# kazuotani14/iLQR

Measured on AMD Instinct MI355X. Metric: iLQR iterations/sec (batch x T timesteps/sec), acrobot T=500 batch=4096, higher is better.
Workload: dtype f64; 1 GPU; acrobot n=4 m=1 T=499 (500 knots), box-QP limits active, FD derivatives + backward/box-QP + 11-alpha search + accept, fixed work; batch_per_gpu=4096, global_batch=4096, T=499, parallelism=batch shards x1, one all_gather of costs

## Files before the change

ilqr_amd/csrc/backward_hex.hpp:

```cpp
#pragma once
#include "solve_tile.hpp"

namespace ilqr {

#ifndef ILQR_COMMIT_ROLLED
#define ILQR_COMMIT_ROLLED 1
#endif

constexpr int HT = 4;
#ifndef ILQR_HEX_SLOT_PAD
#define ILQR_HEX_SLOT_PAD 8
#endif
#ifndef ILQR_HEX_PAIR_PERM
#define ILQR_HEX_PAIR_PERM 1
#endif
#ifndef ILQR_HEX_CAND_T
#define ILQR_HEX_CAND_T 1
#endif
constexpr bool kHexCandT = ILQR_HEX_CAND_T != 0;

template <int NX, int NU, class real, int SLOTS_, bool COMPACT_ = false>
struct HexRing {
  static constexpr bool COMPACT = COMPACT_;
  static constexpr int US = Rec<NX, NU>::SIZE;
  static constexpr int PAIRS = COMPACT ? CompactRec<NX, NU>::PAIRS : (Rec<NX, NU>::SIZE + NU + 1) / 2;
  static constexpr int ROW = 2 * HT;
  static constexpr int PAD = ROW - 2 * TW;
  static constexpr int ELEMS = PAIRS * ROW + ILQR_HEX_SLOT_PAD;
  static constexpr int Z = PAIRS * ROW;
  static_assert(!COMPACT || ILQR_HEX_SLOT_PAD >= ROW, "the compact slot keeps Z in its pad row");
  static_assert(!COMPACT || (NX == 4 && NU == 1), "compact slots: nx = 4, nu = 1");
  static constexpr int SLOTS = SLOTS_;
  static constexpr bool PERM = (ILQR_HEX_PAIR_PERM != 0) && NX == 4 && NU == 1;
  static constexpr int pos(int pair) { return PERM && (!COMPACT || pair < 8) ? hex_pair_pos(pair) : pair; }
};

constexpr int kHexKnotsPerRound = 64 / HT;
constexpr int kHexFullSlots = 24;
template <int NX, int NU, class real, bool COMPACT>
struct HexRingSize {
  using Full = HexRing<NX, NU, real, kHexFullSlots, false>;
  static constexpr int TERM = COMPACT ? ((NX + NX * NX) / 2) * Full::ROW : 0;
  static constexpr int SLOTS = COMPACT ? (kHexFullSlots * Full::ELEMS - TERM) / HexRing<NX, NU, real, 1, COMPACT>::ELEMS : kHexFullSlots;
  static constexpr int LEAD = SLOTS - kHexKnotsPerRound - 1;
  static_assert(SLOTS > LEAD + kHexKnotsPerRound - 1 && LEAD >= 1, "a round must not reach a slot the chain has not left");
  static_assert(SLOTS * HexRing<NX, NU, real, 1, COMPACT>::ELEMS + TERM <= kHexFullSlots * Full::ELEMS, "the pair's records fit the bytes of 24 full slots");
};

template <class real, int N>
struct HexTerm {
  alignas(16) real term[N];
};
template <class real>
struct HexTerm<real, 0> {
  static constexpr real* term = nullptr;
};

template <class real, int NX, int NU, bool COMPACT = false>
struct HexPair : HexTerm<real, HexRingSize<NX, NU, real, COMPACT>::TERM> {
  using Size = HexRingSize<NX, NU, real, COMPACT>;
  using RS = HexRing<NX, NU, real, Size::SLOTS, COMPACT>;
  static constexpr int LEAD = Size::LEAD;
  alignas(16) real ring[RS::SLOTS * RS::ELEMS];
  int rounds_done;
  int consumer_at;
  int passes_started;
  unsigned long long pass_lanes;
};

template <class P>
struct HexGate {
  static constexpr bool kRing = true;
  P& sh;
  const int T, nrounds, N;
  int pass = -1, have = 0;
  int g_next = 0, slot_next = 0, slot_cur = 0;
  __device__ __forceinline__ HexGate(P& s, int T_) : sh(s), T(T_), nrounds((T_ + 1 + kHexKnotsPerRound - 1) / kHexKnotsPerRound), N(nrounds * kHexKnotsPerRound) {}
  __device__ __forceinline__ void begin_pass() {
    pass++;
    have = pass * N;
    g_next = pass * N;
    slot_next = g_next % P::RS::SLOTS;
    __hip_atomic_store(&sh.pass_lanes, __ballot(1), __ATOMIC_RELAXED, __HIP_MEMORY_SCOPE_WORKGROUP);
    __hip_atomic_store(&sh.passes_started, pass + 1, __ATOMIC_RELEASE, __HIP_MEMORY_SCOPE_WORKGROUP);
  }
  __device__ __forceinline__ int slot(int) const { return slot_cur; }
  __device__ __forceinline__ void wait(int) {
    const int G = g_next++;
    slot_cur = slot_next;
    slot_next = (slot_next + 1 == P::RS::SLOTS) ? 0 : slot_next + 1;
    __hip_atomic_store(&sh.consumer_at, G, __ATOMIC_RELAXED, __HIP_MEMORY_SCOPE_WORKGROUP);
    if (G < have) return;
    const int round = pass * nrounds + (G - pass * N) / kHexKnotsPerRound;
    while (__hip_atomic_load(&sh.rounds_done, __ATOMIC_ACQUIRE, __HIP_MEMORY_SCOPE_WORKGROUP) <= round) __builtin_amdgcn_s_sleep(1);
    have = pass * N + ((G - pass * N) / kHexKnotsPerRound + 1) * kHexKnotsPerRound;
  }
  __device__ __forceinline__ void finish() {
    __hip_atomic_store(&sh.consumer_at, 0x3fffffff, __ATOMIC_RELAXED, __HIP_MEMORY_SCOPE_WORKGROUP);
    __hip_atomic_store(&sh.passes_started, -1, __ATOMIC_RELEASE, __HIP_MEMORY_SCOPE_WORKGROUP);
  }
};

__device__ __forceinline__ int hex_first(unsigned long long bal, int t4) {
  return __builtin_ctzll(((bal >> t4) & 0x000F000F000F000Full) | 0x8000000000000000ull);
}
__device__ __forceinline__ void qp1_search_hex(QP1StateT<double>& q, int j, int t4, double step_j0, const double* __restrict__ lds_steps) {
  const double t_x1 = clamp_of(q.x + step_j0 * q.search, q.lo, q.hi);
  const double t_v1 = qp1_value(q, t_x1);
  const bool t_pass = !qp1_armijo_fails(q, t_v1, step_j0);
  const int pp = hex_first(__ballot(t_pass), t4);
  const bool success = pp < 52;
  const int jw = success ? (((pp >> 4) << 2) | (pp & 3)) : 0;
#ifdef ILQR_EXP_NO_STEP_LDS
  q.step = jw == 0 ? 1.0 : 0.6;
#else
  q.step = lds_steps[jw];
#endif
  q.x1 = clamp_of(q.x + q.step * q.search, q.lo, q.hi);
  q.v1 = qp1_value(q, q.x1);
  bool more = p_and(!success, !q.early);
  if (__builtin_expect(__ballot(more) == 0ull, 1)) return;
  {
    const bool stuck = p_and(j >= 1, t_x1 == q.x);
    const int qs = hex_first(__ballot(p_and(stuck, more)), t4);
    if (p_and(more, qs < 52)) {
      q.ls_failed = true;
      more = false;
    }
    if (__ballot(more) == 0ull) return;
  }
  for (int base = 16;; base += 16) {
    const int kn = base + j;
    const double my_step = lds_steps[kn < 104 ? kn : 103];
    const double my_x1 = qp1_trial(q, my_step);
    const double my_v1 = qp1_value(q, my_x1);
    const bool pass = !qp1_armijo_fails(q, my_v1, my_step);
    const bool stuck = p_or(my_step < kMinStep, my_x1 == q.x);
    const int qp = hex_first(__ballot(p_and(pass, more)), t4), qs = hex_first(__ballot(p_and(stuck, more)), t4);
    if (more) {
      if (qp < qs) {
        q.step = lds_steps[base + (((qp >> 4) << 2) | (qp & 3))];
        q.x1 = qp1_trial(q, q.step);
        q.v1 = qp1_value(q, q.x1);
        more = false;
      } else if (qs < 52) {
        q.ls_failed = true;
        more = false;
      }
    }
    if (__ballot(more) == 0ull) return;
  }
}

template <class RS>
__device__ __forceinline__ int hex_pos_rt(int pair) { return RS::pos(pair); }

template <class real>
struct HexStep {
  typedef real pair_t __attribute__((ext_vector_type(2)));
  real F, cxx_rc, cxx_cr, fu_r, cx_r, cxu_r, cxu_c;
  pair_t tail, uw;
};

template <class M, class Gate, class RS>
__device__ __forceinline__ void backward_hex(const BatchViewT<typename M::real>& v, const M& model, const SolverParams& sp, int mode, int tile, int sub,
                                             int lane, const double* __restrict__ lds_steps, Gate& gate, const typename M::real* __restrict__ ring,
                                             const typename M::real* __restrict__ term ) {
  using real = typename M::real;
  using creal = double;
  static_assert(M::NX == 4 && M::NU == 1, "hex chain: nx = 4, nu = 1");
  using R = Rec<4, 1>;
  typedef real real2_t __attribute__((ext_vector_type(2)));
  const int r_ = lane >> 4, t_ = (lane >> 2) & 3, c_ = lane & 3, j16 = 4 * r_ + c_;
  const int t4 = 4 * t_;
  const int l = sub * HT + t_;
  const int b = tile * TW + l;
  if (b >= v.B) return;
  if (mode == 1 && v.status[b] != 0) return;
  const int T = v.T;
  double lambda = v.lambda[b], dlambda = v.dlambda[b];
  const real* __restrict__ ust = v.us + tidx(tile, 0, 0, l, T, 1);
  real* __restrict__ kt = v.kff + tidx(tile, 0, 0, l, T, 1);
  real* __restrict__ Kt = v.Kfb + tidx(tile, 0, 0, l, T, 4);
  typedef const __attribute__((address_space(3))) real lds_cd;
  typedef const __attribute__((address_space(3))) real2_t lds_cd2;
  const creal step_j0 = lds_steps[j16];
  auto mm = [](creal a, creal bb) __attribute__((always_inline)) { return __builtin_amdgcn_mfma_f64_4x4x4f64(a, bb, 0.0, 0, 0, 0); };

  auto load = [&](int t, HexStep<real>& d) __attribute__((always_inline)) {
    gate.wait(t);
    lds_cd* r = (lds_cd*)(ring + gate.slot(t) * RS::ELEMS + t_ * 2);
    auto pair = [&](int e) { return *(lds_cd2*)(r + RS::pos(e >> 1) * RS::ROW); };
    auto one = [&](int e) { return r[hex_pos_rt<RS>(e >> 1) * RS::ROW + (e & 1)]; };
    if constexpr (RS::COMPACT) {
      using C = CompactRec<4, 1>;
      d.F = one(C::FX + r_ + 4 * c_);
      d.fu_r = one(C::FU + r_);
      d.cxx_rc = d.cxx_cr = d.cx_r = d.cxu_r = d.cxu_c = r[RS::Z];
      d.tail = pair(C::CU);
      d.uw = pair(C::US);
      return;
    }
    d.F = one(R::FX + r_ + 4 * c_);
    d.cxx_rc = one(R::CXX + r_ + 4 * c_);
    d.cxx_cr = one(R::CXX + c_ + 4 * r_);
    d.fu_r = one(R::FU + r_);
    d.cx_r = one(R::CX + r_);
    d.cxu_r = one(R::CXU + r_);
    d.cxu_c = one(R::CXU + c_);
    d.tail = pair(R::CU);
    d.uw = pair(RS::US);
  };

  int diverge = 0;
  bool done = false;
  double dV0 = 0, dV1 = 0, gacc = 0;
  auto one_pass = [&]() __attribute__((always_inline)) {
    gate.begin_pass();
    creal V, RVx, kprev;
    const creal lam_r = (creal)lambda;
    {
      gate.wait(T);
      if constexpr (RS::COMPACT) {
        using C = CompactRec<4, 1>;
        lds_cd* r = (lds_cd*)(term + t_ * 2);
        RVx = (creal)r[((C::TERM_CX + r_) >> 1) * RS::ROW + ((C::TERM_CX + r_) & 1)];
        V = (creal)r[((C::TERM_CXX + r_ + 4 * c_) >> 1) * RS::ROW + ((C::TERM_CXX + r_ + 4 * c_) & 1)];
      } else {
      lds_cd* r = (lds_cd*)(ring + gate.slot(T) * RS::ELEMS + t_ * 2);
      RVx = (creal)r[hex_pos_rt<RS>((R::CX + r_) >> 1) * RS::ROW + ((R::CX + r_) & 1)];
      V = (creal)r[hex_pos_rt<RS>((R::CXX + r_ + 4 * c_) >> 1) * RS::ROW + ((R::CXX + r_ + 4 * c_) & 1)];
      }
    }
    kprev = (creal)kt[(unsigned)((T - 1) * TW)];
    __builtin_amdgcn_s_waitcnt(0x0F70);
    dV0 = dV1 = 0;
    diverge = 0;
    gacc = 0;
    real* __restrict__ Kt_i = Kt + (unsigned)(((T - 1) * 4 + c_) * TW);
    real* __restrict__ kt_i = kt + (unsigned)((T - 1) * TW);

    auto step = [&](int i, const HexStep<real>& raw, HexStep<real>& nxt) -> bool {
      const creal F = (creal)raw.F, Rfu = (creal)raw.fu_r;
      const creal cu = (creal)raw.tail.x, cuu = (creal)raw.tail.y, us = (creal)raw.uw.x, usw = (creal)raw.uw.y;
      const creal W = mm(V, F);
      const creal wv = mm(V, Rfu);
      const creal aQu = mm(Rfu, RVx);
      const creal aQx = mm(F, RVx);
      const creal Tm = mm(F, W);
      const creal Tt = mm(W, F);
      const creal aQuu = mm(Rfu, wv);
      const creal aQux_c = mm(Rfu, W);
      const creal aQux_r = mm(W, Rfu);
      const creal Qxx_rc = (creal)raw.cxx_rc + Tm, Qxx_cr = (creal)raw.cxx_cr + Tt;
      const creal Qx_r = (creal)raw.cx_r + aQx;
      const creal Qu = cu + aQu;
      const creal Qux_c = (creal)raw.cxu_c + aQux_c, Qux_r = (creal)raw.cxu_r + aQux_r;
      const creal Quu = cuu + aQuu, QuuF = (cuu + lam_r) + aQuu;
      const creal lo = (creal)model.u_min[0] - us, hi = (creal)model.u_max[0] - us;
      __builtin_amdgcn_sched_barrier(0);
      if (i >= 1) load(i - 1, nxt);
      __builtin_amdgcn_sched_barrier(0);
      creal x;
      int free0;
      creal minv;
      QP1StateT<creal> q1;
      qp1_begin<false>(QuuF, Qu, kprev, lo, hi, q1, false);
      qp1_search_hex(q1, j16, t4, step_j0, lds_steps);
      bool goes_on;
      bool ok = qp1_finish_ok(q1, x, free0, minv, goes_on);
      if (goes_on)
        ok = qp1_continue(
                 q1, [&](QP1StateT<creal>& qs) __attribute__((always_inline)) { qp1_search_hex(qs, j16, t4, step_j0, lds_steps); }, x, free0) >= 1;
      if (!ok) diverge = i;
      const creal k_scale = free0 ? -minv : creal(0);
      const creal K_r = k_scale * Qux_r, K_c = k_scale * Qux_c;
      creal d0 = 0, d1 = 0;
      {
        d0 += x * Qu;
        creal rq = 0;
        rq += (creal(0.5) * x) * Quu;
        d1 += rq * x;
      }
      creal T1_r, T1_c;
      {
        creal acc = 0;
        acc += K_r * Quu;
        T1_r = acc;
      }
      {
        creal acc = 0;
        acc += K_c * Quu;
        T1_c = acc;
      }
      creal Vxn_r, Vn_rc, Vn_cr;
      {
        creal t1 = 0, t2 = 0, t3 = 0;
        t1 += T1_r * x;
        t2 += K_r * Qu;
        t3 += Qux_r * x;
        Vxn_r = ((Qx_r + t1) + t2) + t3;
      }
      {
        creal u1 = 0, u2 = 0, u3 = 0;
        u1 += T1_r * K_c;
        u2 += K_r * Qux_c;
        u3 += Qux_r * K_c;
        Vn_rc = ((Qxx_rc + u1) + u2) + u3;
      }
      {
        creal u1 = 0, u2 = 0, u3 = 0;
        u1 += T1_c * K_r;
        u2 += K_c * Qux_r;
        u3 += Qux_c * K_r;
        Vn_cr = ((Qxx_cr + u1) + u2) + u3;
      }
      V = creal(0.5) * (Vn_rc + Vn_cr);
      RVx = Vxn_r;
      if (ok) {
        dV0 += (double)d0;
        dV1 += (double)d1;
        gacc += (double)(abs_of(x) * usw);
        kprev = (creal)(real)x;
        Kt_i[0] = (real)K_c;
        kt_i[0] = (real)x;
      }
      Kt_i -= 4 * TW;
      kt_i -= TW;
      return ok;
    };

    HexStep<real> A, Bd;
    int i = T - 1;
    load(i, A);
    while (true) {
      if (!step(i, A, Bd)) break;
      if (--i < 0) break;
      if (!step(i, Bd, A)) break;
      if (--i < 0) break;
    }
  };

  while (true) {
    one_pass();
    if (mode == 0) {
      done = (diverge == 0);
      break;
    }
    if (diverge != 0) {
      dlambda = raised_dlambda(dlambda, sp);
      lambda = raised_lambda(lambda, dlambda, sp);
      if (lambda > sp.lambda_max) break;
      continue;
    }
    done = true;
    break;
  }

  double acc = gacc;
  if (!done) {
    __builtin_amdgcn_fence(__ATOMIC_RELEASE, "workgroup");
    __builtin_amdgcn_s_waitcnt(0);
    acc = 0;
    for (int t0 = 0; t0 < T; t0 += 8) {
      real kv[8], uv[8];
#pragma unroll
      for (int jj = 0; jj < 8; jj++) {
        const int t = (t0 + jj < T) ? t0 + jj : T - 1;
        kv[jj] = kt[(size_t)t * TW];
        uv[jj] = ust[(size_t)t * TW];
      }
#pragma unroll
      for (int jj = 0; jj < 8; jj++) {
        const real mx = abs_of(kv[jj]) / (abs_of(uv[jj]) + 1);
        if (t0 + jj < T) acc += (double)mx;
      }
    }
  }
  const double gnorm = acc / T;
  if (j16 == 0) {
    v.dV[b] = dV0;
    v.dV[v.Bp + b] = dV1;
    v.diverge[b] = diverge;
    v.backpass_done[b] = done ? 1 : 0;
    v.gnorm[b] = gnorm;
    if (mode == 1) {
      v.lambda[b] = lambda;
      v.dlambda[b] = dlambda;
      if (!sp.fixed_work && gnorm < sp.tol_grad && lambda < kLambdaConverged) {
        v.status[b] = 1;
        v.iters[b] += 1;
      }
    }
  }
}

template <class M, class MFD, class P>
__device__ __forceinline__ void sweep_backward_hex(const BatchViewT<typename M::real>& v, const M& model, const MFD& fdm, const SolverParams& sp, int mode,
                                                   int force, int tile, P* pairs, const double* __restrict__ lds_steps, int role) {
  using RS = typename P::RS;
  const int lane = threadIdx.x & 63;
  if (threadIdx.x < 4) {
    pairs[threadIdx.x].rounds_done = 0;
    pairs[threadIdx.x].consumer_at = 0;
    pairs[threadIdx.x].passes_started = 0;
  }
  __syncthreads();
  const int T = v.T;
  P& sh = pairs[role & 3];
  if (role < 4) {
    __builtin_amdgcn_s_setprio(3);
    HexGate<P> gate(sh, T);
    backward_hex<M, decltype(gate), RS>(v, model, sp, mode, tile, role, lane, lds_steps, gate, sh.ring, sh.term);
    gate.finish();
    __builtin_amdgcn_s_setprio(0);
  } else {
    const int sub = role - 4;
    const int lp = lane & (HT - 1), ks = lane >> 2;
    const int l = sub * HT + lp;
    const int nrounds = (T + 1 + kHexKnotsPerRound - 1) / kHexKnotsPerRound, N = nrounds * kHexKnotsPerRound;
    for (int pass = 0;; pass++) {
      unsigned long long lanes = ~0ull;
      if (pass > 0) {
        int started;
        while ((started = __hip_atomic_load(&sh.passes_started, __ATOMIC_ACQUIRE, __HIP_MEMORY_SCOPE_WORKGROUP)) >= 0 && started <= pass)
          __builtin_amdgcn_s_sleep(8);
        if (started < 0) break;
        lanes = __hip_atomic_load(&sh.pass_lanes, __ATOMIC_RELAXED, __HIP_MEMORY_SCOPE_WORKGROUP);
      }
      const bool mine = (lanes >> (4 * lp)) & 1ull;
      for (int r = 0; r < nrounds; r++) {
        const int j0 = r * kHexKnotsPerRound, G0 = pass * N + j0;
        while (G0 > __hip_atomic_load(&sh.consumer_at, __ATOMIC_RELAXED, __HIP_MEMORY_SCOPE_WORKGROUP) + P::LEAD) __builtin_amdgcn_s_sleep(4);
        const int started = __hip_atomic_load(&sh.passes_started, __ATOMIC_RELAXED, __HIP_MEMORY_SCOPE_WORKGROUP);
        if ((started < 0) | (started > pass + 1)) break;
        const int t = T - (j0 + ks);
        if (t >= 0 && (pass == 0 || mine)) {
          typename M::real* rs = sh.ring + ((G0 + ks) % RS::SLOTS) * RS::ELEMS + lp * 2;
          if constexpr (RS::COMPACT) {
            if (t == T) rs = sh.term + lp * 2;
          }
          derivatives_of_knot<M, true, MFD, RS::PAD, RS::PERM, RS::COMPACT>(v, model, fdm, force, nullptr, tile, t, l, rs, true);
        }
        __builtin_amdgcn_s_waitcnt(0xC07F);
        if (lane == 0) __hip_atomic_store(&sh.rounds_done, pass * nrounds + r + 1, __ATOMIC_RELEASE, __HIP_MEMORY_SCOPE_WORKGROUP);
      }
    }
  }
}

template <class M, bool CANDT = false>
__device__ __forceinline__ void commit_tile_chunks(const BatchViewT<typename M::real>& v, const M& model, const int* commit_of_lane , int tile) {
  using real = typename M::real;
  constexpr int NX = M::NX, NU = M::NU;
  static_assert(!CANDT || (NX == 4 && NU == 1 && CT == 8 && CG == 4), "grouped candidates: nx = 4, nu = 1");
  const int T = v.T;
  const real dt = (real)v.dt;
  const int ntask = v.nch * TW;
  for (int task = threadIdx.x; task < ntask; task += blockDim.x) {
    const int l = task & (TW - 1), c = task >> 4;
    const int b = tile * TW + l;
    const int ci = (b < v.B) ? commit_of_lane[l] : -1;
    if (ci < 0) continue;
    const int ta = ci * v.ntiles + tile;
    real x[NX], uq[CT][NU];
    if constexpr (CANDT) {
      typedef real real4v __attribute__((ext_vector_type(4)));
      const real4v xv = *reinterpret_cast<const real4v*>(v.cand_x + cand_g_x(ta, c, l, v.nch, NX));
      x[0] = xv.x;
      x[1] = xv.y;
      x[2] = xv.z;
      x[3] = xv.w;
      const real4v u0 = *reinterpret_cast<const real4v*>(v.cand_u + cand_g_u(ta, 2 * c, l, T));
      const real4v u1 = *reinterpret_cast<const real4v*>(v.cand_u + cand_g_u(ta, 2 * c + 1, l, T));
      uq[0][0] = u0.x;
      uq[1][0] = u0.y;
      uq[2][0] = u0.z;
      uq[3][0] = u0.w;
      uq[4][0] = u1.x;
      uq[5][0] = u1.y;
      uq[6][0] = u1.z;
      uq[7][0] = u1.w;
    } else {
#pragma unroll
    for (int i = 0; i < NX; i++) x[i] = v.cand_x[tidx(ta, c, i, l, v.nch, NX)];
#pragma unroll
    for (int q = 0; q < CT; q++) {
      const int tq = (c * CT + q < T) ? c * CT + q : T - 1;
#pragma unroll
      for (int jj = 0; jj < NU; jj++) uq[q][jj] = v.cand_u[tidx(ta, tq, jj, l, T, NU)];
    }
    }
#if ILQR_COMMIT_ROLLED
#pragma unroll 1
    for (int q = 0; q < CT; q++) {
      const int t = c * CT + q;
      if (t > T) break;
#pragma unroll
      for (int i = 0; i < NX; i++) v.xs[tidx(tile, t, i, l, T + 1, NX)] = x[i];
      if (t < T) {
#pragma unroll
        for (int jj = 0; jj < NU; jj++) v.us[tidx(tile, t, jj, l, T, NU)] = uq[0][jj];
        if (q + 1 < CT) {
          real x1[NX];
          integrate_dynamics(model, x, uq[0], dt, x1);
#pragma unroll
          for (int i = 0; i < NX; i++) x[i] = x1[i];
        }
      }
#pragma unroll
      for (int qq = 0; qq + 1 < CT; qq++)
#pragma unroll
        for (int jj = 0; jj < NU; jj++) uq[qq][jj] = uq[qq + 1][jj];
    }
#else
#pragma unroll
    for (int q = 0; q < CT; q++) {
      const int t = c * CT + q;
      if (t <= T) {
#pragma unroll
        for (int i = 0; i < NX; i++) v.xs[tidx(tile, t, i, l, T + 1, NX)] = x[i];
        if (t < T) {
#pragma unroll
          for (int jj = 0; jj < NU; jj++) v.us[tidx(tile, t, jj, l, T, NU)] = uq[q][jj];
          if (q + 1 < CT) {
            real x1[NX];
            integrate_dynamics(model, x, uq[q], dt, x1);
#pragma unroll
            for (int i = 0; i < NX; i++) x[i] = x1[i];
          }
        }
      }
    }
#endif
  }
}

template <class M, class MFD>
__global__ __launch_bounds__(512) __attribute__((amdgpu_waves_per_eu(2, 2))) void k_solve_hex(BatchViewT<typename M::real> v, M model, MFD fdm, AlphaSet alphas,
                                                                                                 SolverParams sp, int n_iters, int force,
                                                                                                 int* __restrict__ commit_idx, int commit_pending,
                                                                                                 long long* __restrict__ phase_ticks) {
  using real = typename M::real;
  using P = HexPair<real, M::NX, M::NU, state_free_running_cost<M>::value>;
  __shared__ P pairs[4];
  __shared__ double steps[104];
  __shared__ double lds_cost[NALPHA * TW];
  __shared__ int tile_running;
  __shared__ int simd_count[4];
  __shared__ int lds_commit[TW];
  if (threadIdx.x < 4) simd_count[threadIdx.x] = 0;
  load_step_table(steps);
  const int wave = (int)(threadIdx.x >> 6);
  int role = wave;
  {
    const int simd = hw_simd_id();
    int slot = 0;
    if ((threadIdx.x & 63) == 0) slot = atomicAdd(&simd_count[simd], 1);
    slot = __shfl(slot, 0, 64);
    __syncthreads();
    if (simd_count[0] == 2 && simd_count[1] == 2 && simd_count[2] == 2 && simd_count[3] == 2) role = simd + 4 * slot;
  }
  const int rwave = (role < 3) ? role : 3;
  const int tile = blockIdx.x;
  constexpr int kShareReals = 4 * ((2 * M::NU + M::NU * M::NX + M::NX + 3) / 4) * TW;
  static_assert(kShareReals <= (int)(sizeof(pairs[0].ring) / sizeof(real)), "a pair's ring holds a wavefront's rollout rows");
  long long t_sweep = 0, t_roll = 0, t0 = 0;
#ifdef ILQR_HEX_SECTIONS
  long long t_sweep_last = 0;
#endif
  const bool timing = (phase_ticks != nullptr) & (threadIdx.x == 0);
  const long long c_begin = timing ? clock64() : 0, w_begin = timing ? wall_clock64() : 0;
  if (commit_pending) {
    commit_tile_chunks<M>(v, model, commit_idx + tile * TW, tile);
    phase_barrier();
  }
  int it = 0;
  for (; it < n_iters; it++) {
    if (timing) t0 = wall_clock64();
    sweep_backward_hex<M, MFD, P>(v, model, fdm, sp, 1, force, tile, pairs, steps, role);
    phase_barrier();
    if (timing) {
      const long long t1 = wall_clock64();
#ifdef ILQR_HEX_SECTIONS
      t_sweep_last = t1 - t0;
#endif
      t_sweep += t1 - t0;
      t0 = t1;
    }
    rollout_tile<M, true, true, kDeepPrefetch<M>, true, true, true, 1, kHexCandT>(v, model, alphas, NALPHA, v.cost_c, 1, sp, commit_idx, tile, lds_cost, it == n_iters - 1, rwave,
                                               pairs[role & 3].ring);
#ifdef ILQR_HEX_SECTIONS
#define ILQR_HEX_MARK(n)                                   \
    if (ILQR_HEX_SECTIONS == n && timing) {                \
      const long long t1 = wall_clock64();                 \
      t_sweep = t_sweep - t_sweep_last + (t1 - t0);        \
      t0 = t1;                                             \
    }
#else
#define ILQR_HEX_MARK(n)
#endif
    ILQR_HEX_MARK(1)
    if (threadIdx.x < TW) lds_commit[threadIdx.x] = commit_idx[tile * TW + threadIdx.x];
    if (threadIdx.x == 0) tile_running = 0;
    phase_barrier();
    ILQR_HEX_MARK(2)
    commit_tile_chunks<M, kHexCandT>(v, model, lds_commit, tile);
    ILQR_HEX_MARK(3)
    phase_barrier();
    if (timing) t_roll += wall_clock64() - t0;
    if (!sp.fixed_work) {
      const int b = tile * TW + (int)threadIdx.x;
      if (threadIdx.x < TW && b < v.B && v.status[b] == 0) tile_running = 1;
      __syncthreads();
      if (!tile_running) {
        it++;
        break;
      }
    }
  }
  if (timing) {
    phase_ticks[5 * tile + 0] += t_sweep;
    phase_ticks[5 * tile + 1] += t_roll;
    phase_ticks[5 * tile + 2] += it;
    phase_ticks[5 * tile + 3] += clock64() - c_begin;
    phase_ticks[5 * tile + 4] += wall_clock64() - w_begin;
  }
}

}
```

ilqr_amd/csrc/rollout.hpp:

```cpp
#pragma once
#include "layout.hpp"

namespace ilqr {

template <class View, class CostOf>
__device__ __forceinline__ void accept_one(const View& v, const SolverParams& sp, int b, CostOf cost_of,
                                           int* __restrict__ commit_idx, bool count_running = true) {
  if (b >= v.Bp) return;
  int commit = -1;
  if (b < v.B && v.status[b] == 0) {
    double lambda = v.lambda[b], dlambda = v.dlambda[b];
    const double cost_s = v.cost[b];
    bool fwd = false;
    double new_cost = 0, dcost = 0;
    int acc = -1;
    if (v.backpass_done[b]) {
      const double dV0 = v.dV[b], dV1 = v.dV[v.Bp + b];
      for (int a = 0; a < NALPHA; a++) {
        const double alpha = kAlpha[a];
        new_cost = cost_of(a);
        dcost = cost_s - new_cost;
        double expected;
        {
#pragma clang fp contract(off)
          expected = -alpha * (dV0 + alpha * dV1);
        }
        double z;
        if (expected > 0)
          z = dcost / expected;
        else
          z = (double)((0.0 < dcost) - (dcost < 0.0));
        if (z > sp.z_min) {
          fwd = true;
          acc = a;
          break;
        }
      }
    }
    int status = 0;
    if (fwd) {
      dlambda = fmin(dlambda / sp.lambda_factor, 1 / sp.lambda_factor);
      lambda = lambda * dlambda * (lambda > sp.lambda_min ? 1.0 : 0.0);
      v.cost[b] = new_cost;
      v.flg_change[b] = 1;
      commit = acc;
      if (!sp.fixed_work && dcost < sp.tol_fun) status = 2;
    } else {
      dlambda = fmax(dlambda * sp.lambda_factor, sp.lambda_factor);
      lambda = fmax(lambda * dlambda, sp.lambda_min);
      v.flg_change[b] = 0;
      if (!sp.fixed_work && lambda > sp.lambda_max) status = 3;
    }
    v.lambda[b] = lambda;
    v.dlambda[b] = dlambda;
    v.alpha_idx[b] = acc;
    const int it = v.iters[b] + 1;
    v.iters[b] = it;
    if (status == 0 && !sp.fixed_work && it >= sp.max_iter) status = 4;
    v.status[b] = status;
    if (status == 0 && count_running) atomicAdd(v.n_running, 1);
  }
  commit_idx[b] = commit;
}
template <class real>
__global__ void k_accept(BatchViewT<real> v, SolverParams sp, int* __restrict__ commit_idx) {
  const int b = blockIdx.x * blockDim.x + threadIdx.x;
  accept_one(v, sp, b, [&](int a) { return v.cost_c[(size_t)a * v.Bp + b]; }, commit_idx);
}

struct AlphaSet {
  double a[NALPHA];
};

#ifndef ILQR_ROLLOUT_UNCLAMPED_FETCH
#define ILQR_ROLLOUT_UNCLAMPED_FETCH 1
#endif
constexpr int kRolloutFetchSlack = 8;
constexpr size_t rollout_fetch_slack_elems(int nx, int nu) { return (size_t)kRolloutFetchSlack * nu * nx * TW; }
template <class M>
constexpr int kDeepPrefetch = (M::NU * M::NX + M::NX + 2 * M::NU <= 10) ? 8 : 4;

constexpr int CG = 4;
static_assert(CT % CG == 0, "a chunk of the commit is a whole number of control groups");
__host__ __device__ inline int cand_groups(int T) { return (T + CT + CG - 1) / CG; }
__host__ __device__ inline size_t cand_g_u(int ta, int grp, int l, int T) { return (((size_t)ta * cand_groups(T) + grp) * TW + l) * CG; }
__host__ __device__ inline size_t cand_g_x(int ta, int c, int l, int nch, int NX) { return (((size_t)ta * nch + c) * TW + l) * NX; }
template <class M, bool GAINS, bool CAND, int PD, bool ACCEPT, bool SHARE = false, bool NOFIX = false, int NG = 1, bool CANDT = false>
__device__ __forceinline__ void rollout_tile(const BatchViewT<typename M::real>& v, const M& model, const AlphaSet& alphas, int n_alpha,
                                             double* __restrict__ cost_out, int mode, const SolverParams& sp,
                                             int* __restrict__ commit_idx, int tile, double* lds_cost, bool count_running = true, int rwave = -1,
                                             typename M::real* share = nullptr) {
  using real = typename M::real;
  constexpr int NX = M::NX, NU = M::NU;
  static_assert(NG == 1 || (SHARE && GAINS && !ACCEPT), "several alpha groups per wavefront: the shared-row rollout of the wide tiles");
  static_assert(!CANDT || (CAND && SHARE && GAINS && NU == 1 && NX == 4 && PD % CG == 0), "grouped candidates: the matrix-core kernel's rollouts (nx = 4, nu = 1)");
  const int wave = (rwave >= 0) ? rwave : (int)(threadIdx.x >> 6);
  const int lane = threadIdx.x & 63;
  const int l = lane & (TW - 1);
  const int a_sub = lane >> 4;
  const int b = tile * TW + l;
  int a[NG];
  bool active[NG];
  bool any_active = false;
  const bool eligible = (b < v.B) && (mode != 1 || (v.status[b < v.B ? b : 0] == 0 && v.backpass_done[b < v.B ? b : 0]));
#pragma unroll
  for (int g = 0; g < NG; g++) {
    a[g] = (wave + g) * 4 + a_sub;
    active[g] = eligible && (a[g] < n_alpha);
    any_active = any_active || active[g];
  }
  const bool run = (SHARE && GAINS) ? (__ballot(any_active) != 0ull) : any_active;
  if (!ACCEPT && !run) return;
  if (run) {
  const int T = v.T;
  real alpha[NG];
#pragma unroll
  for (int g = 0; g < NG; g++) alpha[g] = (real)alphas.a[a[g] < NALPHA ? a[g] : NALPHA - 1];
  const real dt = (real)v.dt;

  real x[NG][NX];
#pragma unroll
  for (int i = 0; i < NX; i++) {
    const real x0i = v.x0[tidx(tile, 0, i, l, 1, NX)];
#pragma unroll
    for (int g = 0; g < NG; g++) x[g][i] = x0i;
  }
  double total[NG];
#pragma unroll
  for (int g = 0; g < NG; g++) total[g] = 0;

  struct StepIn {
    real u[NU], k[GAINS ? NU : 1], K[GAINS ? NU * NX : 1], xnom[GAINS ? NX : 1];
  };
  auto load_step = [&](int t, StepIn& d) __attribute__((always_inline)) {
    t = (t < T) ? t : T - 1;
#pragma unroll
    for (int j = 0; j < NU; j++) d.u[j] = v.us[tidx(tile, t, j, l, T, NU)];
    if (GAINS) {
#pragma unroll
      for (int j = 0; j < NU; j++) d.k[j] = v.kff[tidx(tile, t, j, l, T, NU)];
#pragma unroll
      for (int e = 0; e < NU * NX; e++) d.K[e] = v.Kfb[tidx(tile, t, e, l, T, NU * NX)];
#pragma unroll
      for (int i = 0; i < NX; i++) d.xnom[i] = v.xs[tidx(tile, t, i, l, T + 1, NX)];
    }
  };
  int ta_store[NG];
#pragma unroll
  for (int g = 0; g < NG; g++) ta_store[g] = ((SHARE && CAND && !active[g]) ? NALPHA : a[g]) * v.ntiles + tile;
  typedef real real4v __attribute__((ext_vector_type(4)));
  real pend[NG][CG - 1];
#pragma unroll
  for (int g = 0; g < NG; g++)
#pragma unroll
    for (int q = 0; q < CG - 1; q++) pend[g][q] = 0;
  auto store_group = [&](int g, int t, real last) __attribute__((always_inline)) {
    real4v w;
    w.x = pend[g][0];
    w.y = pend[g][1];
    w.z = pend[g][2];
    w.w = last;
    *reinterpret_cast<real4v*>(v.cand_u + cand_g_u(ta_store[g], t / CG, l, T)) = w;
  };
  auto emit_knot = [&](int g, int t, const real* xx, const real* uu, auto with_u, auto ph) __attribute__((always_inline)) {
    if (SHARE && !CAND && !active[g]) return;
    if constexpr (CANDT) {
      constexpr int p = decltype(ph)::value;
      if (with_u) {
        if constexpr (p == CG - 1)
          store_group(g, t, uu[0]);
        else
          pend[g][p] = uu[0];
      }
      if ((t & (CT - 1)) == 0) {
        real4v w;
        w.x = xx[0];
        w.y = xx[1];
        w.z = xx[2];
        w.w = xx[3];
        *reinterpret_cast<real4v*>(v.cand_x + cand_g_x(ta_store[g], t / CT, l, v.nch, NX)) = w;
      }
    } else if (CAND) {
      const int ta = ta_store[g];
      if (with_u) {
#pragma unroll
        for (int q = 0; q < NU; q++) v.cand_u[tidx(ta, t, q, l, T, NU)] = uu[q];
      }
      if ((t & (CT - 1)) == 0) {
#pragma unroll
        for (int i = 0; i < NX; i++) v.cand_x[tidx(ta, t / CT, i, l, v.nch, NX)] = xx[i];
      }
    } else {
#pragma unroll
      for (int i = 0; i < NX; i++) v.xs[tidx(tile, t, i, l, T + 1, NX)] = xx[i];
      if (with_u) {
#pragma unroll
        for (int q = 0; q < NU; q++) v.us[tidx(tile, t, q, l, T, NU)] = uu[q];
      }
    }
  };
  const WithTrigConsts<M> rmodel(model);
  auto do_step = [&](int t, const StepIn& d, auto ph) __attribute__((always_inline)) {
#pragma unroll
    for (int g = 0; g < NG; g++) {
      real u[NU];
#pragma unroll
      for (int j = 0; j < NU; j++) u[j] = d.u[j];
      if (GAINS) {
#pragma unroll
        for (int j = 0; j < NU; j++) {
          u[j] += d.k[j] * alpha[g];
          real acc = 0;
#pragma unroll
          for (int i = 0; i < NX; i++) acc += d.K[j + NU * i] * (x[g][i] - d.xnom[i]);
          u[j] += acc;
        }
      }
      if (!NOFIX && (sp.fixes & 1)) {
#pragma unroll
        for (int j = 0; j < NU; j++) u[j] = min_of(max_of(u[j], model.u_min[j]), model.u_max[j]);
      }
      emit_knot(g, t, x[g], u, std::true_type(), ph);
      total[g] += (double)model.cost(x[g], u);
      real x1[NX];
      integrate_dynamics(rmodel, x[g], u, dt, x1);
#pragma unroll
      for (int i = 0; i < NX; i++) x[g][i] = x1[i];
    }
  };
  if constexpr (SHARE && GAINS) {
    static_assert(PD % 2 == 0 || PD == 1, "static ring indices");
    static_assert((size_t)PD * NU * NX * TW <= rollout_fetch_slack_elems(NX, NU), "PD knots past the end");
    constexpr int NROWS = 2 * NU + NU * NX + NX;
    constexpr int NLD = (NROWS + 3) / 4;
    struct Raw {
      real r[NLD];
    };
    const real* rbase[NLD];
    unsigned rstride[NLD];
#pragma unroll
    for (int j = 0; j < NLD; j++) {
      const int row = (a_sub + 4 * j < NROWS) ? a_sub + 4 * j : NROWS - 1;
      if (row < NU) {
        rbase[j] = v.us + tidx(tile, 0, row, l, T, NU);
        rstride[j] = NU * TW;
      } else if (row < 2 * NU) {
        rbase[j] = v.kff + tidx(tile, 0, row - NU, l, T, NU);
        rstride[j] = NU * TW;
      } else if (row < 2 * NU + NU * NX) {
        rbase[j] = v.Kfb + tidx(tile, 0, row - 2 * NU, l, T, NU * NX);
        rstride[j] = NU * NX * TW;
      } else {
        rbase[j] = v.xs + tidx(tile, 0, row - 2 * NU - NU * NX, l, T + 1, NX);
        rstride[j] = NX * TW;
      }
    }
    auto fetch = [&](int tt, Raw& d) __attribute__((always_inline)) {
#if !ILQR_ROLLOUT_UNCLAMPED_FETCH
      tt = (tt < T) ? tt : T - 1;
#endif
#pragma unroll
      for (int j = 0; j < NLD; j++) d.r[j] = rbase[j][(size_t)tt * rstride[j]];
    };
    typedef real real2_t __attribute__((ext_vector_type(2)));
    constexpr int NPAIR = (NROWS + 1) / 2;
    real* const mine = share + (((a_sub >> 1) * TW + l) * 2 + (a_sub & 1));
    auto put = [&](const Raw& d) __attribute__((always_inline)) {
#pragma unroll
      for (int j = 0; j < NLD; j++) mine[4 * j * TW] = d.r[j];
    };
    const real2_t* const row0 = reinterpret_cast<const real2_t*>(share + 2 * l);
    auto get = [&](StepIn& d) __attribute__((always_inline)) {
      real rows[2 * NPAIR];
#pragma unroll
      for (int q = 0; q < NPAIR; q++) {
        const real2_t pr = row0[q * TW];
        rows[2 * q] = pr.x;
        rows[2 * q + 1] = pr.y;
      }
#pragma unroll
      for (int j = 0; j < NU; j++) d.u[j] = rows[j];
#pragma unroll
      for (int j = 0; j < NU; j++) d.k[j] = rows[NU + j];
#pragma unroll
      for (int e = 0; e < NU * NX; e++) d.K[e] = rows[2 * NU + e];
#pragma unroll
      for (int i = 0; i < NX; i++) d.xnom[i] = rows[2 * NU + NU * NX + i];
    };
    Raw ring[PD];
#pragma unroll
    for (int d = 0; d < PD; d++) fetch(d, ring[d]);
    StepIn cur, nxt;
    put(ring[0]);
    get(cur);
    auto one = [&](int s_, Raw& free_set, const Raw& next_set, auto ph) __attribute__((always_inline)) {
      put(next_set);
      get(nxt);
      fetch(s_ + PD, free_set);
      do_step(s_, cur, ph);
      cur = nxt;
    };
    int t = 0;
    for (; t + PD <= T; t += PD) {
      static_for<PD>([&](auto dc) __attribute__((always_inline)) {
        constexpr int d = decltype(dc)::value;
        one(t + d, ring[d], ring[(d + 1) % PD], std::integral_constant<int, d % CG>());
      });
    }
    static_for<PD>([&](auto dc) __attribute__((always_inline)) {
      constexpr int d = decltype(dc)::value;
      if (t + d < T) one(t + d, ring[d], ring[(d + 1) % PD], std::integral_constant<int, d % CG>());
    });
  } else {
  StepIn ring[PD];
#pragma unroll
  for (int d = 0; d < PD; d++) load_step(d, ring[d]);
  int t = 0;
  for (; t + PD <= T; t += PD) {
#pragma unroll
    for (int d = 0; d < PD; d++) {
      do_step(t + d, ring[d], std::integral_constant<int, 0>());
      load_step(t + d + PD, ring[d]);
    }
  }
  for (; t < T; t++) {
    StepIn cur;
    load_step(t, cur);
    do_step(t, cur, std::integral_constant<int, 0>());
  }
  }
#pragma unroll
  for (int g = 0; g < NG; g++) {
    {
      real uz[NU];
#pragma unroll
      for (int q = 0; q < NU; q++) uz[q] = 0;
      emit_knot(g, T, x[g], uz, std::false_type(), std::integral_constant<int, 0>());
      if constexpr (CANDT) {
        if (T % CG) store_group(g, T - 1, pend[g][CG - 2]);
      }
    }
    total[g] += (double)model.final_cost(x[g]);
    if (active[g]) {
      cost_out[(size_t)a[g] * v.Bp + b] = total[g];
      if (ACCEPT) lds_cost[a[g] * TW + l] = total[g];
    }
  }
  }
  if constexpr (ACCEPT) {
    __syncthreads();
    if (threadIdx.x < TW)
      accept_one(v, sp, tile * TW + (int)threadIdx.x, [&](int aa) { return lds_cost[aa * TW + threadIdx.x]; }, commit_idx, count_running);
  }
}

template <class M, bool GAINS, bool CAND, int PD = 4, bool ACCEPT = false>
__global__ __launch_bounds__(192) void k_rollout(BatchViewT<typename M::real> v, M model, AlphaSet alphas, int n_alpha,
                                                 double* __restrict__ cost_out, int mode, SolverParams sp,
                                                 int* __restrict__ commit_idx) {
  __shared__ double lds_cost[ACCEPT ? NALPHA * TW : 1];
  rollout_tile<M, GAINS, CAND, PD, ACCEPT>(v, model, alphas, n_alpha, cost_out, mode, sp, commit_idx, (int)blockIdx.x, lds_cost);
}

template <class M, bool CANDT = false>
__device__ __forceinline__ void candidate_knot(const BatchViewT<typename M::real>& v, const M& model, int a, int tile, int t, int l,
                                               typename M::real* x, typename M::real* u) {
  using real = typename M::real;
  constexpr int NX = M::NX, NU = M::NU;
  const int T = v.T, ta = a * v.ntiles + tile, c = t / CT, off = t - c * CT;
#pragma unroll
  for (int i = 0; i < NX; i++) x[i] = CANDT ? v.cand_x[cand_g_x(ta, c, l, v.nch, NX) + i] : v.cand_x[tidx(ta, c, i, l, v.nch, NX)];
  real uq[CT][NU];
#pragma unroll
  for (int q = 0; q < CT; q++) {
    const int tq = (c * CT + q < T) ? c * CT + q : T - 1;
#pragma unroll
    for (int j = 0; j < NU; j++) uq[q][j] = CANDT ? v.cand_u[cand_g_u(ta, tq / CG, l, T) + tq % CG] : v.cand_u[tidx(ta, tq, j, l, T, NU)];
  }
#pragma unroll
  for (int j = 0; j < NU; j++) u[j] = 0.0;
#pragma unroll
  for (int q = 0; q < CT; q++) {
    if (q < off) {
      real x1[NX];
      integrate_dynamics(model, x, uq[q], (real)v.dt, x1);
#pragma unroll
      for (int i = 0; i < NX; i++) x[i] = x1[i];
    }
    if (q == off && t < T) {
#pragma unroll
      for (int j = 0; j < NU; j++) u[j] = uq[q][j];
    }
  }
}

template <class M, bool CANDT = false>
__global__ void k_unpack_cand(BatchViewT<typename M::real> v, M model, int a, double* __restrict__ xs, double* __restrict__ us) {
  using real = typename M::real;
  constexpr int NX = M::NX, NU = M::NU;
  const int T = v.T;
  const size_t n = (size_t)v.B * (T + 1);
  for (size_t i = (size_t)blockIdx.x * blockDim.x + threadIdx.x; i < n; i += (size_t)gridDim.x * blockDim.x) {
    const int t = (int)(i % (T + 1));
    const int b = (int)(i / (T + 1));
    real x[NX], u[NU];
    candidate_knot<M, CANDT>(v, model, a, b / TW, t, b % TW, x, u);
    if (xs)
      for (int e = 0; e < NX; e++) xs[((size_t)b * (T + 1) + t) * NX + e] = (double)x[e];
    if (us && t < T)
      for (int e = 0; e < NU; e++) us[((size_t)b * T + t) * NU + e] = (double)u[e];
  }
}

}
```

Baseline: 4.366 billion trajectory-timesteps/s.

## Roll out all alphas of four trajectories per wavefront and batch commit tasks

The line-search rollout gets a quad mode. Each wavefront handles four trajectories and puts all eleven alphas on separate lanes (44 of 64 lanes), and each lane fetches one shared gain/state row. Four wavefronts now do rollouts instead of three, and the leftover lanes sit idle. The commit pass is also restructured to load two candidate tasks before integrating either, so global loads overlap with the serial dynamics steps, at the cost of more registers per thread.

```diff
diff --git a/ilqr_amd/csrc/backward_hex.hpp b/ilqr_amd/csrc/backward_hex.hpp
--- a/ilqr_amd/csrc/backward_hex.hpp
+++ b/ilqr_amd/csrc/backward_hex.hpp
@@ -6,6 +6,11 @@
 #ifndef ILQR_COMMIT_ROLLED
 #define ILQR_COMMIT_ROLLED 1
 #endif
+
+#ifndef ILQR_COMMIT_BATCH
+#define ILQR_COMMIT_BATCH 2
+#endif
+constexpr int kCommitBatch = ILQR_COMMIT_BATCH;
 
 constexpr int HT = 4;
 #ifndef ILQR_HEX_SLOT_PAD
@@ -18,6 +23,10 @@
 #define ILQR_HEX_CAND_T 1
 #endif
 constexpr bool kHexCandT = ILQR_HEX_CAND_T != 0;
+#ifndef ILQR_HEX_QUAD_ROLLOUT
+#define ILQR_HEX_QUAD_ROLLOUT 1
+#endif
+constexpr bool kHexQuadRollout = ILQR_HEX_QUAD_ROLLOUT != 0;
 
 template <int NX, int NU, class real, int SLOTS_, bool COMPACT_ = false>
 struct HexRing {
@@ -454,16 +463,27 @@
   using real = typename M::real;
   constexpr int NX = M::NX, NU = M::NU;
   static_assert(!CANDT || (NX == 4 && NU == 1 && CT == 8 && CG == 4), "grouped candidates: nx = 4, nu = 1");
+  static_assert(HT == kQuad, "a chain wavefront rolls out its own sub-tile");
   const int T = v.T;
   const real dt = (real)v.dt;
   const int ntask = v.nch * TW;
-  for (int task = threadIdx.x; task < ntask; task += blockDim.x) {
+  struct Task {
+    int l, c;
+    real x[NX], uq[CT][NU];
+  };
+  auto load = [&](int task, Task& k) __attribute__((always_inline)) {
+    k.l = 0;
+    k.c = -1;
+    if (task < 0) return;
     const int l = task & (TW - 1), c = task >> 4;
     const int b = tile * TW + l;
     const int ci = (b < v.B) ? commit_of_lane[l] : -1;
-    if (ci < 0) continue;
+    if (ci < 0) return;
+    k.l = l;
+    k.c = c;
     const int ta = ci * v.ntiles + tile;
-    real x[NX], uq[CT][NU];
+    real* const x = k.x;
+    real(*const uq)[NU] = k.uq;
     if constexpr (CANDT) {
       typedef real real4v __attribute__((ext_vector_type(4)));
       const real4v xv = *reinterpret_cast<const real4v*>(v.cand_x + cand_g_x(ta, c, l, v.nch, NX));
@@ -491,6 +511,12 @@
       for (int jj = 0; jj < NU; jj++) uq[q][jj] = v.cand_u[tidx(ta, tq, jj, l, T, NU)];
     }
     }
+  };
+  auto steps = [&](Task& k) __attribute__((always_inline)) {
+    if (k.c < 0) return;
+    const int l = k.l, c = k.c;
+    real* const x = k.x;
+    real(*const uq)[NU] = k.uq;
 #if ILQR_COMMIT_ROLLED
 #pragma unroll 1
     for (int q = 0; q < CT; q++) {
@@ -533,6 +559,13 @@
       }
     }
 #endif
+  };
+  for (int first = ntask - 1 - (int)threadIdx.x; first >= 0; first -= kCommitBatch * (int)blockDim.x) {
+    Task k[kCommitBatch];
+#pragma unroll
+    for (int j = 0; j < kCommitBatch; j++) load(first - j * (int)blockDim.x, k[j]);
+#pragma unroll
+    for (int j = 0; j < kCommitBatch; j++) steps(k[j]);
   }
 }
 
@@ -561,7 +594,7 @@
     __syncthreads();
     if (simd_count[0] == 2 && simd_count[1] == 2 && simd_count[2] == 2 && simd_count[3] == 2) role = simd + 4 * slot;
   }
-  const int rwave = (role < 3) ? role : 3;
+  const int rwave = kHexQuadRollout ? ((role < 4) ? role : 4) : ((role < 3) ? role : 3);
   const int tile = blockIdx.x;
   constexpr int kShareReals = 4 * ((2 * M::NU + M::NU * M::NX + M::NX + 3) / 4) * TW;
   static_assert(kShareReals <= (int)(sizeof(pairs[0].ring) / sizeof(real)), "a pair's ring holds a wavefront's rollout rows");
@@ -588,7 +621,7 @@
       t_sweep += t1 - t0;
       t0 = t1;
     }
-    rollout_tile<M, true, true, kDeepPrefetch<M>, true, true, true, 1, kHexCandT>(v, model, alphas, NALPHA, v.cost_c, 1, sp, commit_idx, tile, lds_cost, it == n_iters - 1, rwave,
+    rollout_tile<M, true, true, kDeepPrefetch<M>, true, true, true, 1, kHexCandT, kHexQuadRollout>(v, model, alphas, NALPHA, v.cost_c, 1, sp, commit_idx, tile, lds_cost, it == n_iters - 1, rwave,
                                                pairs[role & 3].ring);
 #ifdef ILQR_HEX_SECTIONS
 #define ILQR_HEX_MARK(n)                                   \
diff --git a/ilqr_amd/csrc/quad_lanes.hpp b/ilqr_amd/csrc/quad_lanes.hpp
--- /dev/null
+++ b/ilqr_amd/csrc/quad_lanes.hpp
@@ -0,0 +1,32 @@
+#pragma once
+#include "common.hpp"
+
+namespace ilqr {
+
+constexpr int kQuad = 4;
+
+constexpr int quad_rollout_lanes(int nalpha) { return kQuad * nalpha; }
+constexpr int quad_lane_alpha(int lane) { return lane / kQuad; }
+constexpr int quad_lane_q(int lane) { return lane % kQuad; }
+constexpr int quad_traj(int s, int q) { return kQuad * s + q; }
+constexpr int quad_fetch_row(int lane, int nrows) { return lane / kQuad < nrows ? lane / kQuad : nrows - 1; }
+
+constexpr int rollout_share_slot(int row, int l) { return ((row >> 1) * TW + l) * 2 + (row & 1); }
+constexpr int rollout_share_pair(int p, int l) { return (p * TW + l) * 2; }
+constexpr int rollout_rows(int nx, int nu) { return 2 * nu + nu * nx + nx; }
+
+enum { ROW_US = 0, ROW_KFF = 1, ROW_KFB = 2, ROW_XS = 3 };
+struct RowSource {
+  int array, elem, E, S;
+};
+constexpr RowSource rollout_row_source(int row, int nx, int nu, int T) {
+  return row < nu                 ? RowSource{ROW_US, row, nu, T}
+         : row < 2 * nu           ? RowSource{ROW_KFF, row - nu, nu, T}
+         : row < 2 * nu + nu * nx ? RowSource{ROW_KFB, row - 2 * nu, nu * nx, T}
+                                  : RowSource{ROW_XS, row - 2 * nu - nu * nx, nx, T + 1};
+}
+constexpr size_t rollout_row_elem(const RowSource& r, int tile, int tt, int l) {
+  return ((((size_t)tile * r.S) * r.E + r.elem) * TW + l) + (size_t)tt * r.E * TW;
+}
+
+}
diff --git a/ilqr_amd/csrc/rollout.hpp b/ilqr_amd/csrc/rollout.hpp
--- a/ilqr_amd/csrc/rollout.hpp
+++ b/ilqr_amd/csrc/rollout.hpp
@@ -1,5 +1,6 @@
 #pragma once
 #include "layout.hpp"
+#include "quad_lanes.hpp"
 
 namespace ilqr {
 
@@ -85,7 +86,7 @@
 __host__ __device__ inline int cand_groups(int T) { return (T + CT + CG - 1) / CG; }
 __host__ __device__ inline size_t cand_g_u(int ta, int grp, int l, int T) { return (((size_t)ta * cand_groups(T) + grp) * TW + l) * CG; }
 __host__ __device__ inline size_t cand_g_x(int ta, int c, int l, int nch, int NX) { return (((size_t)ta * nch + c) * TW + l) * NX; }
-template <class M, bool GAINS, bool CAND, int PD, bool ACCEPT, bool SHARE = false, bool NOFIX = false, int NG = 1, bool CANDT = false>
+template <class M, bool GAINS, bool CAND, int PD, bool ACCEPT, bool SHARE = false, bool NOFIX = false, int NG = 1, bool CANDT = false, bool QUAD = false>
 __device__ __forceinline__ void rollout_tile(const BatchViewT<typename M::real>& v, const M& model, const AlphaSet& alphas, int n_alpha,
                                              double* __restrict__ cost_out, int mode, const SolverParams& sp,
                                              int* __restrict__ commit_idx, int tile, double* lds_cost, bool count_running = true, int rwave = -1,
@@ -93,10 +94,13 @@
   using real = typename M::real;
   constexpr int NX = M::NX, NU = M::NU;
   static_assert(NG == 1 || (SHARE && GAINS && !ACCEPT), "several alpha groups per wavefront: the shared-row rollout of the wide tiles");
+  static_assert(!QUAD || (SHARE && GAINS && NG == 1 && quad_rollout_lanes(NALPHA) <= 64 && kQuad * rollout_rows(NX, NU) <= quad_rollout_lanes(NALPHA)),
+                "quad rollouts: every alpha of four trajectories in one wavefront, whose lanes also fetch the quad's rows");
   static_assert(!CANDT || (CAND && SHARE && GAINS && NU == 1 && NX == 4 && PD % CG == 0), "grouped candidates: the matrix-core kernel's rollouts (nx = 4, nu = 1)");
   const int wave = (rwave >= 0) ? rwave : (int)(threadIdx.x >> 6);
   const int lane = threadIdx.x & 63;
-  const int l = lane & (TW - 1);
+  const int l = QUAD ? quad_traj(wave & 3, quad_lane_q(lane)) : lane & (TW - 1);
+  const bool idle = QUAD && lane >= quad_rollout_lanes(NALPHA);
   const int a_sub = lane >> 4;
   const int b = tile * TW + l;
   int a[NG];
@@ -105,13 +109,13 @@
   const bool eligible = (b < v.B) && (mode != 1 || (v.status[b < v.B ? b : 0] == 0 && v.backpass_done[b < v.B ? b : 0]));
 #pragma unroll
   for (int g = 0; g < NG; g++) {
-    a[g] = (wave + g) * 4 + a_sub;
-    active[g] = eligible && (a[g] < n_alpha);
+    a[g] = QUAD ? quad_lane_alpha(lane) : (wave + g) * 4 + a_sub;
+    active[g] = eligible && (a[g] < n_alpha) && (!QUAD || wave < 4);
     any_active = any_active || active[g];
   }
   const bool run = (SHARE && GAINS) ? (__ballot(any_active) != 0ull) : any_active;
   if (!ACCEPT && !run) return;
-  if (run) {
+  if (run && !idle) {
   const int T = v.T;
   real alpha[NG];
 #pragma unroll
@@ -232,7 +236,8 @@
     static_assert(PD % 2 == 0 || PD == 1, "static ring indices");
     static_assert((size_t)PD * NU * NX * TW <= rollout_fetch_slack_elems(NX, NU), "PD knots past the end");
     constexpr int NROWS = 2 * NU + NU * NX + NX;
-    constexpr int NLD = (NROWS + 3) / 4;
+    static_assert(NROWS == rollout_rows(NX, NU), "quad_lanes.hpp counts the same rows");
+    constexpr int NLD = QUAD ? 1 : (NROWS + 3) / 4;
     struct Raw {
       real r[NLD];
     };
@@ -240,7 +245,7 @@
     unsigned rstride[NLD];
 #pragma unroll
     for (int j = 0; j < NLD; j++) {
-      const int row = (a_sub + 4 * j < NROWS) ? a_sub + 4 * j : NROWS - 1;
+      const int row = QUAD ? quad_fetch_row(lane, NROWS) : (a_sub + 4 * j < NROWS) ? a_sub + 4 * j : NROWS - 1;
       if (row < NU) {
         rbase[j] = v.us + tidx(tile, 0, row, l, T, NU);
         rstride[j] = NU * TW;
@@ -264,12 +269,12 @@
     };
     typedef real real2_t __attribute__((ext_vector_type(2)));
     constexpr int NPAIR = (NROWS + 1) / 2;
-    real* const mine = share + (((a_sub >> 1) * TW + l) * 2 + (a_sub & 1));
+    real* const mine = share + (QUAD ? rollout_share_slot(quad_fetch_row(lane, NROWS), l) : rollout_share_slot(a_sub, l));
     auto put = [&](const Raw& d) __attribute__((always_inline)) {
 #pragma unroll
       for (int j = 0; j < NLD; j++) mine[4 * j * TW] = d.r[j];
     };
-    const real2_t* const row0 = reinterpret_cast<const real2_t*>(share + 2 * l);
+    const real2_t* const row0 = reinterpret_cast<const real2_t*>(share + rollout_share_pair(0, l));
     auto get = [&](StepIn& d) __attribute__((always_inline)) {
       real rows[2 * NPAIR];
 #pragma unroll
```

After: 4.503 billion trajectory-timesteps/s, median of 6. 1.03x the previous value.
